# RookieJunChen/FullSubNet-plus

Hardware: AMD Instinct MI355X
Metric: STFT frames/sec (257-bin, 2 s clips), FullSubNet+ forward (higher is better)
Workload: dtype f32

## Files before the change

### fullsubnet_plus_amd/csrc/lstm.hip

```cpp
#include <cstring>

#include "fsnp_common.h"
#include "lstm_common.h"

namespace fsnp {

template <int EX>
__host__ __device__ __forceinline__ int e_frag_index(int e, int k) {
    return ((((k >> 3) * 2) + (k & 1)) * EX + e) * 4 + ((k >> 1) & 3);
}

struct WStream {
    __amdgpu_buffer_rsrc_t rsrc;
    int voff;
};
template <int NT>
__device__ __forceinline__ float4 wload(const WStream& ws, int g, int n) {
    const auto v = __builtin_amdgcn_raw_buffer_load_b128(ws.rsrc, ws.voff, (g * NT + n) * 1024, 0);
    return __builtin_bit_cast(float4, v);
}

template <int NT, int EX>
__device__ __forceinline__ void mfma_groups(f32x16 (&acc)[NT], float (&accx)[EX > 0 ? EX : 1][NT], float4 (&b)[NT],
                                            const float4* __restrict__ A, const float4* __restrict__ AE, int ngroups,
                                            const WStream& ws, int& gnext, int groups_total) {
    float4 a = A[0];
    float4 ae[EX > 0 ? EX : 1];
#pragma unroll
    for (int e = 0; e < EX; ++e) ae[e] = AE[e];
    for (int g = 0; g < ngroups; ++g) {
        const int gn = (g + 1 < ngroups ? g + 1 : g);
        const float4 an = A[gn * 64];
        float4 aen[EX > 0 ? EX : 1];
#pragma unroll
        for (int e = 0; e < EX; ++e) aen[e] = AE[gn * 2 * EX + e];
        if constexpr (EX == 0) {
#pragma unroll
            for (int n = 0; n < NT; ++n) {
                acc[n] = __builtin_amdgcn_mfma_f32_32x32x2f32(a.x, b[n].x, acc[n], 0, 0, 0);
                acc[n] = __builtin_amdgcn_mfma_f32_32x32x2f32(a.y, b[n].y, acc[n], 0, 0, 0);
                acc[n] = __builtin_amdgcn_mfma_f32_32x32x2f32(a.z, b[n].z, acc[n], 0, 0, 0);
                acc[n] = __builtin_amdgcn_mfma_f32_32x32x2f32(a.w, b[n].w, acc[n], 0, 0, 0);
                b[n] = wload<NT>(ws, gnext, n);
                __builtin_amdgcn_sched_barrier(0);
            }
        } else {
            constexpr int HALF = NT / 2;
#pragma unroll
            for (int hb = 0; hb < NT; hb += HALF) {
#pragma unroll
                for (int n = hb; n < hb + HALF; ++n) {
                    acc[n] = __builtin_amdgcn_mfma_f32_32x32x2f32(a.x, b[n].x, acc[n], 0, 0, 0);
                    acc[n] = __builtin_amdgcn_mfma_f32_32x32x2f32(a.y, b[n].y, acc[n], 0, 0, 0);
                    acc[n] = __builtin_amdgcn_mfma_f32_32x32x2f32(a.z, b[n].z, acc[n], 0, 0, 0);
                    acc[n] = __builtin_amdgcn_mfma_f32_32x32x2f32(a.w, b[n].w, acc[n], 0, 0, 0);
                }
                __builtin_amdgcn_sched_barrier(0);
#pragma unroll
                for (int n = hb; n < hb + HALF; ++n)
#pragma unroll
                    for (int e = 0; e < EX; ++e) {
                        float v = accx[e][n];
                        v = fmaf(ae[e].x, b[n].x, v);
                        v = fmaf(ae[e].y, b[n].y, v);
                        v = fmaf(ae[e].z, b[n].z, v);
                        accx[e][n] = fmaf(ae[e].w, b[n].w, v);
                    }
                __builtin_amdgcn_sched_barrier(0);
#pragma unroll
                for (int n = hb; n < hb + HALF; ++n) b[n] = wload<NT>(ws, gnext, n);
                __builtin_amdgcn_sched_barrier(0);
            }
        }
        gnext = (gnext + 1 == groups_total) ? 0 : gnext + 1;
        a = an;
#pragma unroll
        for (int e = 0; e < EX; ++e) ae[e] = aen[e];
    }
}

__device__ __forceinline__ unsigned short bf16_bits(float v) {
    const unsigned u = __float_as_uint(v);
    return (unsigned short)((u + 0x7FFFu + ((u >> 16) & 1u)) >> 16);
}
__host__ __device__ __forceinline__ int a_frag_index_bf16(int row, int k) {
    return (((k >> 4) * 64) + (((k >> 3) & 1) * 32) + row) * 8 + (k & 7);
}

template <int ST, int UW, int HBLO = 0>
__device__ __forceinline__ void lstm_cell(f32x16 (&acc)[4 * ST], f32x2 (&c)[ST][8], float* __restrict__ Hs, int wave,
                                          int lane, unsigned short* __restrict__ Hb = nullptr) {
#pragma unroll
    for (int s = 0; s < ST; ++s) {
        const int k = wave * UW + s * 32 + (lane & 31);
        const int kbase = (((k >> 3) * 64) + ((k & 1) * 32)) * 4 + ((k >> 1) & 3);
#pragma unroll
        for (int r = 0; r < 16; r += 2) {
            auto rd = [](float v) {
                if constexpr (ST > 1) { float o; asm("v_accvgpr_read_b32 %0, %1" : "=v"(o) : "a"(v)); return o; }
                else return v;
            };
            const f32x2 h = lstm_cell_pair(f32x2{rd(acc[s][r]), rd(acc[s][r + 1])}, f32x2{rd(acc[ST + s][r]), rd(acc[ST + s][r + 1])},
                                           f32x2{rd(acc[2 * ST + s][r]), rd(acc[2 * ST + s][r + 1])},
                                           f32x2{rd(acc[3 * ST + s][r]), rd(acc[3 * ST + s][r + 1])}, c[s][r >> 1]);
            const int row = (r & 3) + 8 * (r >> 2) + 4 * (lane >> 5);
            Hs[kbase + row * 4] = h.x;
            Hs[kbase + (row + 1) * 4] = h.y;
            if (Hb) {
                const unsigned short hx = bf16_bits(h.x), hy = bf16_bits(h.y);
                Hb[a_frag_index_bf16(row, k)] = hx; Hb[a_frag_index_bf16(row + 1, k)] = hy;
                if constexpr (HBLO > 0) {
                    Hb[HBLO + a_frag_index_bf16(row, k)] = bf16_bits(h.x - __uint_as_float((unsigned)hx << 16));
                    Hb[HBLO + a_frag_index_bf16(row + 1, k)] = bf16_bits(h.y - __uint_as_float((unsigned)hy << 16));
                }
            }
        }
    }
}

using bf16x8 = __attribute__((ext_vector_type(8))) __bf16;
template <int NT, int EX, int ALO>
__device__ __forceinline__ void mfma_groups_bf16(f32x16 (&acc)[NT], float (&accx)[EX > 0 ? EX : 1][NT], float4 (&b)[NT],
                                                 const float4* __restrict__ A, const float4* __restrict__ AE, int nsteps,
                                                 const WStream& ws, int& gnext, int groups_total, int lane) {
    float4 a = A[0], al = A[ALO];
    for (int g = 0; g < nsteps; ++g) {
        const float4 an = A[(g + 1 < nsteps ? g + 1 : g) * 64], aln = A[ALO + (g + 1 < nsteps ? g + 1 : g) * 64];
        float4 he[EX > 0 ? EX : 1][2];
        if constexpr (EX > 0) {
            const int kg = 2 * g + (lane >> 5);
#pragma unroll
            for (int e = 0; e < EX; ++e) { he[e][0] = AE[(kg * 2 + 0) * EX + e]; he[e][1] = AE[(kg * 2 + 1) * EX + e]; }
        }
#pragma unroll
        for (int n = 0; n < NT; ++n) {
            if constexpr (EX > 0) {
                const unsigned w0 = __float_as_uint(b[n].x), w1 = __float_as_uint(b[n].y), w2 = __float_as_uint(b[n].z),
                               w3 = __float_as_uint(b[n].w);
#pragma unroll
                for (int e = 0; e < EX; ++e) {
                    float v = accx[e][n];
                    v = fmaf(he[e][0].x, __uint_as_float(w0 << 16), v);
                    v = fmaf(he[e][1].x, __uint_as_float(w0 & 0xFFFF0000u), v);
                    v = fmaf(he[e][0].y, __uint_as_float(w1 << 16), v);
                    v = fmaf(he[e][1].y, __uint_as_float(w1 & 0xFFFF0000u), v);
                    v = fmaf(he[e][0].z, __uint_as_float(w2 << 16), v);
                    v = fmaf(he[e][1].z, __uint_as_float(w2 & 0xFFFF0000u), v);
                    v = fmaf(he[e][0].w, __uint_as_float(w3 << 16), v);
                    accx[e][n] = fmaf(he[e][1].w, __uint_as_float(w3 & 0xFFFF0000u), v);
                }
            }
            acc[n] = __builtin_amdgcn_mfma_f32_32x32x16_bf16(__builtin_bit_cast(bf16x8, a), __builtin_bit_cast(bf16x8, b[n]),
                                                             acc[n], 0, 0, 0);
            if constexpr (ALO > 0)
                acc[n] = __builtin_amdgcn_mfma_f32_32x32x16_bf16(__builtin_bit_cast(bf16x8, al), __builtin_bit_cast(bf16x8, b[n]),
                                                                 acc[n], 0, 0, 0);
            b[n] = wload<NT>(ws, gnext, n);
            __builtin_amdgcn_sched_barrier(0);
        }
        gnext = (gnext + 1 == groups_total) ? 0 : gnext + 1;
        a = an; al = aln;
    }
}

template <int ST, int UW, int EX, int NT>
__device__ __forceinline__ void lstm_cell_extra(float (&accx)[EX > 0 ? EX : 1][NT], float (&cx)[EX > 0 ? EX : 1][ST],
                                                const float* __restrict__ bias, float* __restrict__ He, int wave,
                                                int lane) {
#pragma unroll
    for (int e = 0; e < EX; ++e)
#pragma unroll
        for (int s = 0; s < ST; ++s) {
            float g4[4];
#pragma unroll
            for (int q = 0; q < 4; ++q) {
                const float v = accx[e][q * ST + s];
                g4[q] = v + __shfl_xor(v, 32) + (bias ? bias[(q * ST + s) * 32] : 0.0f);
            }
            const float cn = fast_sigmoid(g4[1]) * cx[e][s] + fast_sigmoid(g4[0]) * fast_tanh(g4[2]);
            cx[e][s] = cn;
            const float h = fast_sigmoid(g4[3]) * fast_tanh(cn);
            if (lane < 32) He[e_frag_index<EX>(e, wave * UW + s * 32 + lane)] = h;
        }
}

template <int HID, int KX, int OUT, int EX, bool PROF, int NW, bool BF>
__global__ __launch_bounds__(64 * NW) __attribute__((amdgpu_waves_per_eu(NW / 4, NW / 4)))
void lstm2_fc_kernel(LstmWeights w, LstmArgs a) {
    static_assert(OUT == 2, "FC lane mapping assumes output_size == 2");
    static_assert(EX >= 0 && EX <= 4, "at most 4 VALU rows per tile (one FC wave per extra row)");
    static_assert(NW % 4 == 0 && NW >= 4, "whole waves per SIMD");
    constexpr int NTHR = 64 * NW;
    constexpr int UW = HID / NW, ST = UW / 32, NT = 4 * ST;
    static_assert(UW % 32 == 0 && UW * NW == HID, "hidden/NW must be a multiple of 32");
    constexpr int KGX = KX / 8, KGH = HID / 8, KG0 = KGX + KGH;
    constexpr int KSB = HID / 16;
    constexpr int KG1 = BF ? KGH + KSB : 2 * KGH, KGT = KG0 + KG1;
    static_assert(KGH % 4 == 0, "FC k-split");
    static_assert(!BF || HID % 16 == 0, "bf16 k-steps");
    constexpr int RT = 32 + EX;
    constexpr int EXA = EX > 0 ? EX : 1;

    extern __shared__ __attribute__((aligned(16))) unsigned char smem_raw[];
    float4* Xs = reinterpret_cast<float4*>(smem_raw);
    float4* H0s = Xs + KGX * 64;
    float4* H1s = H0s + KGH * 64;
    float4* XEs = H1s + KGH * 64;
    float4* HE0s = XEs + KGX * 2 * EX;
    float4* HE1s = HE0s + KGH * 2 * EX;
    float4* Wfc4 = HE1s + KGH * 2 * EX;
    RowDesc* rows_s = reinterpret_cast<RowDesc*>(Wfc4 + OUT * KGH * 2);
    constexpr int BL = BF ? 1 : 2;
    constexpr bool HILO = BF && EX == 0;
    float* Bs = reinterpret_cast<float*>(rows_s + RT);
    float4* H0b = reinterpret_cast<float4*>(Bs + BL * NW * NT * 32);

    const int tid = threadIdx.x;
    const int lane = tid & 63;
    const int wave = __builtin_amdgcn_readfirstlane(tid >> 6);
    const int slot0 = blockIdx.x * RT;
    const int Tp = a.Tp;

    __shared__ unsigned long long clk_s[2];
    if (a.clk != nullptr && tid == 0) {
        clk_s[1] = __builtin_amdgcn_s_memrealtime();
        clk_s[0] = __builtin_amdgcn_s_memtime();
        if (blockIdx.x == 0) { a.clk[0] = clk_s[0]; a.clk[1] = clk_s[1]; a.clk[4] = 0ull; a.clk[5] = 0ull; a.clk[6] = ~0ull; }
    }

    for (int i = tid; i < (KGX + 2 * KGH) * (64 + 2 * EX); i += NTHR) Xs[i] = make_float4(0.f, 0.f, 0.f, 0.f);
    for (int i = tid; i < OUT * KGH * 2; i += NTHR) {
        const int o = i / (KGH * 2), kg = (i >> 1) % KGH, kh = i & 1;
        const float* wr = w.wfc + (size_t)o * HID + kg * 8 + kh;
        Wfc4[i] = make_float4(wr[0], wr[2], wr[4], wr[6]);
    }
    if (tid < RT) rows_s[tid] = a.rows[slot0 + tid];
    for (int i = tid; i < BL * NW * NT * 32; i += NTHR) {
        const int col = i & 31, n = (i >> 5) % NT, wv = (i / (32 * NT)) % NW, layer = BF ? 1 : i / (32 * NT * NW);
        Bs[i] = w.bias[layer * 4 * HID + (n / ST) * HID + wv * UW + (n % ST) * 32 + col];
    }
    __syncthreads();
    if constexpr (BF) {
        if (tid < 32) reinterpret_cast<float*>(Xs)[a_frag_index(tid, w.NIN)] = 1.0f;
        if (EX > 0 && tid < EX) reinterpret_cast<float*>(XEs)[e_frag_index<EXA>(tid, w.NIN)] = 1.0f;
    }

    const bool dense = a.dense != nullptr;
    const float* __restrict__ gbase = dense ? a.dense : a.att_mag;
    const int gstep = dense ? w.NIN : a.FP;
    auto plan = [&](const RowDesc& rd, int j) -> int {
        if (!rd.valid || j >= w.NIN) return -1;
        if (dense) return rd.b * Tp * w.NIN + j;
        return sb_feature_offset(j, rd.f, rd.b * Tp * a.FP, a.F, a.NSBN, a.NFBN, a.fb_rel, a.fb_branch_stride);
    };
    auto row_md = [&](const RowDesc& rd, int slot, NormMD& md, const NormMD*& md_row) {
        md.m = 0.0f; md.d = 1.0f; md_row = nullptr;
        if (dense || !rd.valid) return;
        if (a.md_row != nullptr) md_row = a.md_row + (size_t)slot * Tp;
        else md = a.md_utt[rd.b];
    };
    constexpr int JSTEP = NTHR / 32, NG = (KX + JSTEP - 1) / JSTEP;
    const int grow = tid & 31;
    int goff[NG], xdst[NG];
    NormMD md; const NormMD* md_row;
    {
        const RowDesc rd = rows_s[grow];
#pragma unroll
        for (int i = 0; i < NG; ++i) {
            const int j = (tid >> 5) + JSTEP * i;
            goff[i] = (j < KX && !(BF && j == w.NIN)) ? plan(rd, j) : -2;
            xdst[i] = a_frag_index(grow, j < KX ? j : 0);
        }
        row_md(rd, slot0 + grow, md, md_row);
    }
    int goffx = -1, xdstx = 0;
    NormMD mdx = {0.0f, 1.0f}; const NormMD* mdx_row = nullptr;
    bool havex = EX > 0 && tid < EX * KX;
    if (BF && havex && tid % KX == w.NIN) havex = false;
    if (havex) {
        const int e = tid / KX, j = tid % KX;
        const RowDesc rd = rows_s[32 + e];
        goffx = plan(rd, j);
        xdstx = e_frag_index<EXA>(e, j);
        row_md(rd, slot0 + 32 + e, mdx, mdx_row);
    }

    float* Xf = reinterpret_cast<float*>(Xs);
    float* XEf = reinterpret_cast<float*>(XEs);
    {
        const NormMD m0 = md_row ? md_row[0] : md;
#pragma unroll
        for (int i = 0; i < NG; ++i)
            if (goff[i] != -2) Xf[xdst[i]] = goff[i] >= 0 ? (gbase[goff[i]] - m0.m) / m0.d : 0.0f;
        if (havex) {
            const NormMD mx = mdx_row ? mdx_row[0] : mdx;
            XEf[xdstx] = goffx >= 0 ? (gbase[goffx] - mx.m) / mx.d : 0.0f;
        }
    }

    const float* __restrict__ bias_l0 = BF ? nullptr : Bs + ((0 * NW + wave) * NT) * 32 + (lane & 31);
    const float* __restrict__ bias_l1 = Bs + (((BL - 1) * NW + wave) * NT) * 32 + (lane & 31);
    f32x2 c0[ST][8], c1[ST][8];
    float cx0[EXA][ST], cx1[EXA][ST];
#pragma unroll
    for (int s = 0; s < ST; ++s) {
#pragma unroll
        for (int r = 0; r < 8; ++r) { c0[s][r] = f32x2{0.0f, 0.0f}; c1[s][r] = f32x2{0.0f, 0.0f}; }
#pragma unroll
        for (int e = 0; e < EXA; ++e) { cx0[e][s] = 0.0f; cx1[e][s] = 0.0f; }
    }

    WStream ws;
    ws.rsrc = __builtin_amdgcn_make_buffer_rsrc(const_cast<float*>(w.wpack) + (size_t)wave * KGT * NT * 256, 0,
                                                KGT * NT * 1024, 0x00020000);
    ws.voff = lane * 16;
    float4 breg[NT];
#pragma unroll
    for (int n = 0; n < NT; ++n) breg[n] = wload<NT>(ws, 0, n);
    int gnext = 1;
    auto run_groups = [&](f32x16 (&acc_)[NT], float (&accx_)[EXA][NT], const float4* A_, const float4* AE_, int ng) {
        mfma_groups<NT, EX>(acc_, accx_, breg, A_, AE_, ng, ws, gnext, KGT);
    };

    const int fc_row = (wave & 3) * 8 + (lane & 7);
    const int fc_o = (lane >> 3) & 1;
    const int fc_kp = lane >> 4;
    const RowDesc fc_rd = rows_s[fc_row];
    const RowDesc fcx_rd = (EX > 0 && wave < EX) ? rows_s[32 + (wave < EX ? wave : 0)] : RowDesc{0, 0, 0, 0};

    auto fc_store = [&](int t_of_h) {
      if (wave < 4) {
        constexpr int KGP = KGH / 4;
        float sum = 0.0f;
#pragma unroll 4
        for (int kk = 0; kk < KGP; ++kk) {
            const int kg = fc_kp * KGP + kk;
#pragma unroll
            for (int kh = 0; kh < 2; ++kh) {
                const float4 h4 = H1s[kg * 64 + kh * 32 + fc_row];
                const float4 w4 = Wfc4[(fc_o * KGH + kg) * 2 + kh];
                sum += h4.x * w4.x + h4.y * w4.y + h4.z * w4.z + h4.w * w4.w;
            }
        }
        sum += __shfl_xor(sum, 16);
        sum += __shfl_xor(sum, 32);
        if (fc_kp == 0 && fc_rd.valid && t_of_h >= a.LA)
            a.out[(size_t)fc_rd.out_off + (size_t)fc_o * a.out_stride_o + (t_of_h - a.LA)] = apply_act(sum + w.bfc[fc_o], a.act);
      }
        if (EX > 0 && wave < EX) {
            const int o = lane >> 5;
            const float* he = reinterpret_cast<const float*>(HE1s);
            float sx = 0.0f;
#pragma unroll 4
            for (int i = 0; i < HID / 32; ++i) {
                const int k = (lane & 31) + 32 * i;
                sx += he[e_frag_index<EXA>(wave, k)] * w.wfc[o * HID + k];
            }
#pragma unroll
            for (int m = 16; m > 0; m >>= 1) sx += __shfl_xor(sx, m);
            if ((lane & 31) == 0 && fcx_rd.valid && t_of_h >= a.LA)
                a.out[(size_t)fcx_rd.out_off + (size_t)o * a.out_stride_o + (t_of_h - a.LA)] = apply_act(sx + w.bfc[o], a.act);
        }
    };

    const float4* AEx = XEs + (lane >> 5) * EX;
    const float4* AEh0 = HE0s + (lane >> 5) * EX;
    const float4* AEh1 = HE1s + (lane >> 5) * EX;

    __syncthreads();

    unsigned long long* prof = nullptr;
    int prof_stride = 0;
    if constexpr (PROF) {
        const bool rec = blockIdx.x == 0 && tid == 0;
        prof = a.prof + (rec ? 0 : (size_t)Tp * 8 + (size_t)blockIdx.x * 256 + tid);
        prof_stride = rec ? 8 : 0;
    }
#define FSNP_STAMP(i) do { if constexpr (PROF) prof[t * prof_stride + (prof_stride ? (i) : 0)] = __builtin_amdgcn_s_memtime(); } while (0)

    for (int t = 0; t < Tp; ++t) {
        FSNP_STAMP(0);
        float xr[NG], xrx = 0.0f;
        NormMD mdn = md, mdxn = mdx;
        const bool have_next = (t + 1 < Tp);
        if (have_next) {
            if (md_row) mdn = md_row[t + 1];
#pragma unroll
            for (int i = 0; i < NG; ++i) xr[i] = goff[i] >= 0 ? gbase[goff[i] + (t + 1) * gstep] : 0.0f;
            if (havex) {
                if (mdx_row) mdxn = mdx_row[t + 1];
                xrx = goffx >= 0 ? gbase[goffx + (t + 1) * gstep] : 0.0f;
            }
        }

        f32x16 acc[NT];
        float accx[EXA][NT];
#pragma unroll
        for (int n = 0; n < NT; ++n) {
#pragma unroll
            for (int r = 0; r < 16; ++r) acc[n][r] = BF ? 0.0f : bias_l0[n * 32];
#pragma unroll
            for (int e = 0; e < EXA; ++e) accx[e][n] = 0.0f;
        }
        run_groups(acc, accx, Xs + lane, AEx, KG0);
        FSNP_STAMP(1);
        __syncthreads();
        FSNP_STAMP(2);
        lstm_cell<ST, UW, HILO ? KSB * 64 * 8 : 0>(acc, c0, reinterpret_cast<float*>(H0s), wave, lane, BF ? reinterpret_cast<unsigned short*>(H0b) : nullptr);
        if (EX > 0) lstm_cell_extra<ST, UW, EX, NT>(accx, cx0, bias_l0, reinterpret_cast<float*>(HE0s), wave, lane);
        if (have_next) {
#pragma unroll
            for (int i = 0; i < NG; ++i)
                if (goff[i] != -2) Xf[xdst[i]] = goff[i] >= 0 ? (xr[i] - mdn.m) / mdn.d : 0.0f;
            if (havex) XEf[xdstx] = goffx >= 0 ? (xrx - mdxn.m) / mdxn.d : 0.0f;
        }
        if (t > 0) fc_store(t - 1);
        FSNP_STAMP(3);
        __syncthreads();
        FSNP_STAMP(4);
#pragma unroll
        for (int n = 0; n < NT; ++n) {
#pragma unroll
            for (int r = 0; r < 16; ++r) acc[n][r] = bias_l1[n * 32];
#pragma unroll
            for (int e = 0; e < EXA; ++e) accx[e][n] = 0.0f;
        }
        run_groups(acc, accx, H1s + lane, AEh1, KGH);
        if constexpr (BF) mfma_groups_bf16<NT, EX, HILO ? KSB * 64 : 0>(acc, accx, breg, H0b + lane, HE0s, KSB, ws, gnext, KGT, lane);
        else run_groups(acc, accx, H0s + lane, AEh0, KGH);
        FSNP_STAMP(5);
        __syncthreads();
        FSNP_STAMP(6);
        lstm_cell<ST, UW>(acc, c1, reinterpret_cast<float*>(H1s), wave, lane);
        if (EX > 0) lstm_cell_extra<ST, UW, EX, NT>(accx, cx1, bias_l1, reinterpret_cast<float*>(HE1s), wave, lane);
        FSNP_STAMP(7);
    }
#undef FSNP_STAMP
    __syncthreads();
    fc_store(Tp - 1);
    if (a.clk != nullptr && tid == 0) {
        const unsigned long long m1 = __builtin_amdgcn_s_memtime(), r1 = __builtin_amdgcn_s_memrealtime();
        if (blockIdx.x == 0) { a.clk[2] = m1; a.clk[3] = r1; }
        atomicMax(a.clk + 4, r1 - clk_s[1]);
        atomicMax(a.clk + 5, m1 - clk_s[0]);
        atomicMin(a.clk + 6, r1 - clk_s[1]);
    }
}

size_t lstm_pack_floats(int H, int KX, int NW) {
    const int NT = 4 * (H / NW / 32);
    const int KGT = KX / 8 + H / 8 + 2 * (H / 8);
    return (size_t)NW * KGT * NT * 64 * 4;
}

void lstm_pack_weights(int H, int NIN, int KX, int NW, const float* wih0, const float* whh0, const float* wih1,
                       const float* whh1, float* wpack) {
    const int UW = H / NW, ST = UW / 32, NT = 4 * ST;
    const int KGX = KX / 8, KGH = H / 8, KG0 = KGX + KGH, KGT = KG0 + 2 * KGH;
    for (int wv = 0; wv < NW; ++wv)
        for (int g = 0; g < KGT; ++g)
            for (int n = 0; n < NT; ++n)
                for (int lane = 0; lane < 64; ++lane)
                    for (int p = 0; p < 4; ++p) {
                        const int gate = n / ST, s = n % ST;
                        const int wrow = gate * H + wv * UW + s * 32 + (lane & 31);
                        float v = 0.0f;
                        if (g < KG0) {
                            const int k = 8 * g + 2 * p + (lane >> 5);
                            if (k < KX) { if (k < NIN) v = wih0[(size_t)wrow * NIN + k]; }
                            else v = whh0[(size_t)wrow * H + (k - KX)];
                        } else {
                            const int k = 8 * (g - KG0) + 2 * p + (lane >> 5);
                            if (k < H) v = whh1[(size_t)wrow * H + k];
                            else v = wih1[(size_t)wrow * H + (k - H)];
                        }
                        wpack[((((size_t)wv * KGT + g) * NT + n) * 64 + lane) * 4 + p] = v;
                    }
}

size_t lstm_pack_floats_bf16ih(int H, int KX, int NW) {
    const int NT = 4 * (H / NW / 32);
    const int KGT = KX / 8 + H / 8 + H / 8 + H / 16;
    return (size_t)NW * KGT * NT * 64 * 4;
}

static unsigned short host_bf16(float v) {
    unsigned u;
    memcpy(&u, &v, 4);
    return (unsigned short)((u + 0x7FFFu + ((u >> 16) & 1u)) >> 16);
}

void lstm_pack_weights_bf16ih(int H, int NIN, int KX, int NW, const float* wih0, const float* whh0, const float* wih1,
                              const float* whh1, const float* bias0, float* wpack) {
    const int UW = H / NW, ST = UW / 32, NT = 4 * ST;
    const int KGX = KX / 8, KGH = H / 8, KG0 = KGX + KGH, KSB = H / 16, KGT = KG0 + KGH + KSB;
    for (int wv = 0; wv < NW; ++wv)
        for (int g = 0; g < KGT; ++g)
            for (int n = 0; n < NT; ++n)
                for (int lane = 0; lane < 64; ++lane) {
                    const int gate = n / ST, s = n % ST;
                    const int wrow = gate * H + wv * UW + s * 32 + (lane & 31);
                    float* dst = wpack + ((((size_t)wv * KGT + g) * NT + n) * 64 + lane) * 4;
                    if (g < KG0 + KGH) {
                        for (int p = 0; p < 4; ++p) {
                            float v = 0.0f;
                            if (g < KG0) {
                                const int k = 8 * g + 2 * p + (lane >> 5);
                                if (k < KX) { if (k < NIN) v = wih0[(size_t)wrow * NIN + k]; else if (k == NIN) v = bias0[wrow]; }
                                else v = whh0[(size_t)wrow * H + (k - KX)];
                            } else {
                                const int k = 8 * (g - KG0) + 2 * p + (lane >> 5);
                                v = whh1[(size_t)wrow * H + k];
                            }
                            dst[p] = v;
                        }
                    } else {
                        const int ks = g - KG0 - KGH;
                        unsigned short* d16 = reinterpret_cast<unsigned short*>(dst);
                        for (int j = 0; j < 8; ++j) d16[j] = host_bf16(wih1[(size_t)wrow * H + 16 * ks + 8 * (lane >> 5) + j]);
                    }
                }
}

template <int EX, int NW, bool BF, int KX, int HID = 384>
static void launch_lstm_ex(const LstmWeights& w, const LstmArgs& a, hipStream_t s) {
    constexpr int OUT = 2;
    constexpr int KGX = KX / 8, KGH = HID / 8, NT = 4 * (HID / NW / 32);
    const size_t smem = (size_t)(KGX + 2 * KGH) * (64 + 2 * EX) * 16 + (size_t)OUT * KGH * 2 * 16 +
                        (32 + EX) * sizeof(RowDesc) + (size_t)(BF ? 1 : 2) * NW * NT * 32 * 4 + (BF ? (size_t)(EX == 0 ? 2 : 1) * (HID / 16) * 64 * 16 : 0);
    LstmWeights wv = w;
    wv.wpack = BF ? (NW == 12 ? w.wpack_bf[1] : w.wpack_bf[0]) : (NW == 12 ? w.wpack12 : w.wpack);
    if constexpr (KX == 40 && HID == 384) {
        if (a.prof != nullptr) {
            auto kern = lstm2_fc_kernel<HID, KX, OUT, EX, true, NW, BF>;
            (void)hipFuncSetAttribute(reinterpret_cast<const void*>(kern), hipFuncAttributeMaxDynamicSharedMemorySize, (int)smem);
            hipLaunchKernelGGL(kern, dim3(a.num_tiles), dim3(64 * NW), smem, s, wv, a);
            return;
        }
    }
    auto kern = lstm2_fc_kernel<HID, KX, OUT, EX, false, NW, BF>;
    static PerDeviceOnce attr_once;
    attr_once.run([&] { (void)hipFuncSetAttribute(reinterpret_cast<const void*>(kern), hipFuncAttributeMaxDynamicSharedMemorySize, (int)smem); });
    hipLaunchKernelGGL(kern, dim3(a.num_tiles), dim3(64 * NW), smem, s, wv, a);
}

template <int NW, bool BF, int KX>
static void launch_lstm_nw(const LstmWeights& w, const LstmArgs& a, hipStream_t s) {
    switch (a.ex) {
        case 0: launch_lstm_ex<0, NW, BF, KX>(w, a, s); break;
        case 1: launch_lstm_ex<1, NW, BF, KX>(w, a, s); break;
        case 2: launch_lstm_ex<2, NW, BF, KX>(w, a, s); break;
        default: launch_lstm_ex<4, NW, BF, KX>(w, a, s); break;
    }
}

void launch_lstm(const LstmWeights& w, const LstmArgs& a, hipStream_t s) {
    if (a.num_tiles <= 0) return;
    const int waves = w.waves != 0 ? w.waves : (a.ex > 0 ? 12 : 4);
    if (w.H == 256) {
        if (w.KX == 64) launch_lstm_ex<0, 4, false, 64, 256>(w, a, s);
        else launch_lstm_ex<0, 4, false, 40, 256>(w, a, s);
        return;
    }
    if (w.KX == 64) {
        if (waves == 12) launch_lstm_nw<12, false, 64>(w, a, s);
        else launch_lstm_nw<4, false, 64>(w, a, s);
    } else if (w.ih_bf16) {
        if (waves == 12) launch_lstm_nw<12, true, 40>(w, a, s);
        else launch_lstm_nw<4, true, 40>(w, a, s);
    } else {
        if (waves == 12) launch_lstm_nw<12, false, 40>(w, a, s);
        else launch_lstm_nw<4, false, 40>(w, a, s);
    }
}

template <int ST, int UW, int HID, bool LOAD>
__device__ __forceinline__ void stream_state_io(f32x2 (&c0)[ST][8], f32x2 (&c1)[ST][8], float* __restrict__ H0, float* __restrict__ H1,
                                                const RowDesc* __restrict__ rows_s, float* __restrict__ state, long slot_stride, int done,
                                                int wave, int lane) {
#pragma unroll
    for (int r = 0; r < 16; ++r) {
        const int row = (r & 3) + 8 * (r >> 2) + 4 * (lane >> 5);
        const RowDesc rd = rows_s[row];
        const bool on = LOAD ? rd.valid > 0 : rd.valid == done;
        float* __restrict__ p = state + (size_t)rd.b * slot_stride + (size_t)rd.f * 4 * HID;
#pragma unroll
        for (int s = 0; s < ST; ++s) {
            const int k = wave * UW + s * 32 + (lane & 31);
            const int hi = (((k >> 3) * 64) + ((k & 1) * 32)) * 4 + ((k >> 1) & 3) + row * 4;
            if constexpr (LOAD) {
                H0[hi] = on ? p[k] : 0.0f;
                c0[s][r >> 1][r & 1] = on ? p[HID + k] : 0.0f;
                H1[hi] = on ? p[2 * HID + k] : 0.0f;
                c1[s][r >> 1][r & 1] = on ? p[3 * HID + k] : 0.0f;
            } else if (on) {
                p[k] = H0[hi];
                p[HID + k] = c0[s][r >> 1][r & 1];
                p[2 * HID + k] = H1[hi];
                p[3 * HID + k] = c1[s][r >> 1][r & 1];
            }
        }
    }
}

template <int HID, int KX>
__global__ __launch_bounds__(256) __attribute__((amdgpu_waves_per_eu(1, 1)))
void lstm2_fc_stream_kernel(LstmWeights w, LstmArgs a) {
    constexpr int NW = 4, NTHR = 256, OUT = 2;
    constexpr int UW = HID / NW, ST = UW / 32, NT = 4 * ST;
    constexpr int KGX = KX / 8, KGH = HID / 8, KG0 = KGX + KGH, KGT = KG0 + 2 * KGH;
    static_assert(UW % 32 == 0 && KGH % 4 == 0, "hidden/4 must be a multiple of 32");

    extern __shared__ __attribute__((aligned(16))) unsigned char smem_raw[];
    float4* Xs = reinterpret_cast<float4*>(smem_raw);
    float4* H0s = Xs + KGX * 64;
    float4* H1s = H0s + KGH * 64;
    float4* Wfc4 = H1s + KGH * 64;
    RowDesc* rows_s = reinterpret_cast<RowDesc*>(Wfc4 + OUT * KGH * 2);
    float* Bs = reinterpret_cast<float*>(rows_s + 32);

    const int tid = threadIdx.x;
    const int lane = tid & 63;
    const int wave = __builtin_amdgcn_readfirstlane(tid >> 6);
    const int slot0 = blockIdx.x * 32;
    const int Tp = a.Tp;

    for (int i = tid; i < (KGX + 2 * KGH) * 64; i += NTHR) Xs[i] = make_float4(0.f, 0.f, 0.f, 0.f);
    for (int i = tid; i < OUT * KGH * 2; i += NTHR) {
        const int o = i / (KGH * 2), kg = (i >> 1) % KGH, kh = i & 1;
        const float* wr = w.wfc + (size_t)o * HID + kg * 8 + kh;
        Wfc4[i] = make_float4(wr[0], wr[2], wr[4], wr[6]);
    }
    if (tid < 32) rows_s[tid] = a.rows[slot0 + tid];
    for (int i = tid; i < 2 * NW * NT * 32; i += NTHR) {
        const int col = i & 31, n = (i >> 5) % NT, wv = (i / (32 * NT)) % NW, layer = i / (32 * NT * NW);
        Bs[i] = w.bias[layer * 4 * HID + (n / ST) * HID + wv * UW + (n % ST) * 32 + col];
    }
    __syncthreads();

    int nsteps = 0, cmin = 1 << 30;
    for (int r = 0; r < 32; ++r) {
        const int v = rows_s[r].valid;
        nsteps = v > nsteps ? v : nsteps;
        if (v > 0) cmin = v < cmin ? v : cmin;
    }
    nsteps = __builtin_amdgcn_readfirstlane(nsteps);
    const bool mixed = __builtin_amdgcn_readfirstlane(cmin < nsteps ? 1 : 0) != 0;
    if (nsteps <= 0) return;

    constexpr int JSTEP = NTHR / 32, NG = (KX + JSTEP - 1) / JSTEP;
    const int grow = tid & 31;
    int goff[NG], xdst[NG];
    const float* __restrict__ gbase = a.att_mag;
    const int gstep = a.FP;
    const NormMD* md_row;
    {
        const RowDesc rd = rows_s[grow];
#pragma unroll
        for (int i = 0; i < NG; ++i) {
            const int j = (tid >> 5) + JSTEP * i;
            goff[i] = j >= KX ? -2 : (rd.valid > 0 && j < w.NIN)
                          ? sb_feature_offset(j, rd.f, rd.b * Tp * a.FP, a.F, a.NSBN, a.NFBN, a.fb_rel, a.fb_branch_stride) : -1;
            xdst[i] = a_frag_index(grow, j < KX ? j : 0);
        }
        md_row = a.md_row + (size_t)(slot0 + grow) * Tp;
    }
    float* Xf = reinterpret_cast<float*>(Xs);
    {
        const NormMD m0 = rows_s[grow].valid > 0 ? md_row[0] : NormMD{0.0f, 1.0f};
#pragma unroll
        for (int i = 0; i < NG; ++i)
            if (goff[i] != -2) Xf[xdst[i]] = goff[i] >= 0 ? (gbase[goff[i]] - m0.m) / m0.d : 0.0f;
    }

    const float* __restrict__ bias_l0 = Bs + ((0 * NW + wave) * NT) * 32 + (lane & 31);
    const float* __restrict__ bias_l1 = Bs + ((1 * NW + wave) * NT) * 32 + (lane & 31);
    f32x2 c0[ST][8], c1[ST][8];
    stream_state_io<ST, UW, HID, true>(c0, c1, reinterpret_cast<float*>(H0s), reinterpret_cast<float*>(H1s), rows_s, a.st_sb, a.st_stride, 0,
                                       wave, lane);

    WStream ws;
    ws.rsrc = __builtin_amdgcn_make_buffer_rsrc(const_cast<float*>(w.wpack) + (size_t)wave * KGT * NT * 256, 0, KGT * NT * 1024, 0x00020000);
    ws.voff = lane * 16;
    float4 breg[NT];
#pragma unroll
    for (int n = 0; n < NT; ++n) breg[n] = wload<NT>(ws, 0, n);
    int gnext = 1;
    float accx[1][NT];
    auto run_groups = [&](f32x16 (&acc_)[NT], const float4* A_, int ng) {
        mfma_groups<NT, 0>(acc_, accx, breg, A_, A_, ng, ws, gnext, KGT);
    };

    const int fc_row = (wave & 3) * 8 + (lane & 7);
    const int fc_o = (lane >> 3) & 1;
    const int fc_kp = lane >> 4;
    const RowDesc fc_rd = rows_s[fc_row];
    auto fc_store = [&](int t_of_h) {
        constexpr int KGP = KGH / 4;
        float sum = 0.0f;
#pragma unroll 4
        for (int kk = 0; kk < KGP; ++kk) {
            const int kg = fc_kp * KGP + kk;
#pragma unroll
            for (int kh = 0; kh < 2; ++kh) {
                const float4 h4 = H1s[kg * 64 + kh * 32 + fc_row];
                const float4 w4 = Wfc4[(fc_o * KGH + kg) * 2 + kh];
                sum += h4.x * w4.x + h4.y * w4.y + h4.z * w4.z + h4.w * w4.w;
            }
        }
        sum += __shfl_xor(sum, 16);
        sum += __shfl_xor(sum, 32);
        if (fc_kp == 0 && t_of_h < fc_rd.valid)
            a.out[(size_t)fc_rd.out_off + (size_t)fc_o * a.out_stride_o + t_of_h] = apply_act(sum + w.bfc[fc_o], a.act);
    };

    __syncthreads();

    for (int t = 0; t < nsteps; ++t) {
        float xr[NG];
        NormMD mdn = {0.0f, 1.0f};
        const bool have_next = (t + 1 < nsteps);
        if (have_next) {
            if (rows_s[grow].valid > 0) mdn = md_row[t + 1];
#pragma unroll
            for (int i = 0; i < NG; ++i) xr[i] = goff[i] >= 0 ? gbase[goff[i] + (t + 1) * gstep] : 0.0f;
        }

        f32x16 acc[NT];
#pragma unroll
        for (int n = 0; n < NT; ++n)
#pragma unroll
            for (int r = 0; r < 16; ++r) acc[n][r] = bias_l0[n * 32];
        run_groups(acc, Xs + lane, KG0);
        __syncthreads();
        lstm_cell<ST, UW>(acc, c0, reinterpret_cast<float*>(H0s), wave, lane);
        if (have_next) {
#pragma unroll
            for (int i = 0; i < NG; ++i)
                if (goff[i] != -2) Xf[xdst[i]] = goff[i] >= 0 ? (xr[i] - mdn.m) / mdn.d : 0.0f;
        }
        if (t > 0) fc_store(t - 1);
        __syncthreads();
#pragma unroll
        for (int n = 0; n < NT; ++n)
#pragma unroll
            for (int r = 0; r < 16; ++r) acc[n][r] = bias_l1[n * 32];
        run_groups(acc, H1s + lane, KGH);
        run_groups(acc, H0s + lane, KGH);
        __syncthreads();
        lstm_cell<ST, UW>(acc, c1, reinterpret_cast<float*>(H1s), wave, lane);
        if (t + 1 == nsteps || mixed)
            stream_state_io<ST, UW, HID, false>(c0, c1, reinterpret_cast<float*>(H0s), reinterpret_cast<float*>(H1s), rows_s, a.st_sb,
                                                a.st_stride, t + 1, wave, lane);
    }
    __syncthreads();
    fc_store(nsteps - 1);
}

template <int HID, int KX>
static void launch_lstm_stream_one(const LstmWeights& w, const LstmArgs& a, hipStream_t s) {
    constexpr int KGX = KX / 8, KGH = HID / 8, NT = 4 * (HID / 4 / 32);
    const size_t smem = (size_t)(KGX + 2 * KGH) * 64 * 16 + (size_t)2 * KGH * 2 * 16 + 32 * sizeof(RowDesc) + (size_t)2 * 4 * NT * 32 * 4;
    auto kern = lstm2_fc_stream_kernel<HID, KX>;
    static PerDeviceOnce attr_once;
    attr_once.run([&] { (void)hipFuncSetAttribute(reinterpret_cast<const void*>(kern), hipFuncAttributeMaxDynamicSharedMemorySize, (int)smem); });
    hipLaunchKernelGGL(kern, dim3(a.num_tiles), dim3(256), smem, s, w, a);
}

bool lstm_stream_available(const LstmWeights& w) {
    return !w.gru && w.OUT == 2 && (w.H == 384 || w.H == 256) && (w.KX == 40 || w.KX == 64) && w.wpack != nullptr;
}

void launch_lstm_stream(const LstmWeights& w, const LstmArgs& a, hipStream_t s) {
    if (a.num_tiles <= 0) return;
    if (w.H == 256) { if (w.KX == 64) launch_lstm_stream_one<256, 64>(w, a, s); else launch_lstm_stream_one<256, 40>(w, a, s); }
    else if (w.KX == 64) launch_lstm_stream_one<384, 64>(w, a, s);
    else launch_lstm_stream_one<384, 40>(w, a, s);
}

LstmPlan plan_lstm_tiles(int num_rows, int num_cus) {
    LstmPlan p{};
    if (num_rows <= 32 * num_cus) {
        p.ex = 0; p.num_tiles = cdiv(num_rows, 32);
    } else {
        const int cand[4] = {0, 1, 2, 4};
        int best_rounds = 1 << 30;
        for (int i = 0; i < 4; ++i) {
            const int rounds = cdiv(cdiv(num_rows, 32 + cand[i]), num_cus);
            if (rounds < best_rounds) { best_rounds = rounds; p.ex = cand[i]; }
        }
        p.num_tiles = best_rounds * num_cus;
    }
    p.rows_per_slot_tile = 32 + p.ex;
    return p;
}

}
```

Baseline: 147,200.

## Skip zero-padded input K-groups in LSTM MFMA passes and skip zero h0 at t=0

Replaces the generic rotating MFMA group loop with explicit passes that compute only the input K-groups actually occupied by NIN features, issuing a partial group for the remainder. At the first timestep it also skips the recurrent H contributions, which are known zero. Weight prefetch indices are remapped so the streamed B fragments follow the new irregular group order. This cuts wasted MFMAs and weight loads on padded columns, at the cost of more complex index logic and the risk of mismatched weight/activation groups.

New measurement: 147,100 (median of 5 runs). Within noise of the previous version (-0.1%).

```diff
diff --git a/fullsubnet_plus_amd/csrc/lstm.hip b/fullsubnet_plus_amd/csrc/lstm.hip
--- a/fullsubnet_plus_amd/csrc/lstm.hip
+++ b/fullsubnet_plus_amd/csrc/lstm.hip
@@ -77,6 +77,55 @@
 #pragma unroll
         for (int e = 0; e < EX; ++e) ae[e] = aen[e];
     }
+}
+
+template <int NT>
+__device__ __forceinline__ void mfma_group(f32x16 (&acc)[NT], float4 (&b)[NT], const float4& a, const WStream& ws, int gload) {
+#pragma unroll
+    for (int n = 0; n < NT; ++n) {
+        acc[n] = __builtin_amdgcn_mfma_f32_32x32x2f32(a.x, b[n].x, acc[n], 0, 0, 0);
+        acc[n] = __builtin_amdgcn_mfma_f32_32x32x2f32(a.y, b[n].y, acc[n], 0, 0, 0);
+        acc[n] = __builtin_amdgcn_mfma_f32_32x32x2f32(a.z, b[n].z, acc[n], 0, 0, 0);
+        acc[n] = __builtin_amdgcn_mfma_f32_32x32x2f32(a.w, b[n].w, acc[n], 0, 0, 0);
+        b[n] = wload<NT>(ws, gload, n);
+        __builtin_amdgcn_sched_barrier(0);
+    }
+}
+template <int NT>
+__device__ __forceinline__ void mfma_group_part(f32x16 (&acc)[NT], float4 (&b)[NT], const float4& a, const WStream& ws, int gload,
+                                                int live) {
+#pragma unroll
+    for (int n = 0; n < NT; ++n) {
+        acc[n] = __builtin_amdgcn_mfma_f32_32x32x2f32(a.x, b[n].x, acc[n], 0, 0, 0);
+        if (live > 1) acc[n] = __builtin_amdgcn_mfma_f32_32x32x2f32(a.y, b[n].y, acc[n], 0, 0, 0);
+        if (live > 2) acc[n] = __builtin_amdgcn_mfma_f32_32x32x2f32(a.z, b[n].z, acc[n], 0, 0, 0);
+        if (live > 3) acc[n] = __builtin_amdgcn_mfma_f32_32x32x2f32(a.w, b[n].w, acc[n], 0, 0, 0);
+        b[n] = wload<NT>(ws, gload, n);
+        __builtin_amdgcn_sched_barrier(0);
+    }
+}
+template <int NT, class GroupOf, class AidxOf>
+__device__ __forceinline__ void mfma_pass(f32x16 (&acc)[NT], float4 (&b)[NT], float4& a, const float4* __restrict__ A, int ibeg,
+                                          int iend, GroupOf group_of, AidxOf aidx_of, const WStream& ws) {
+    int i = ibeg;
+    {
+        typedef float f32x4_t __attribute__((ext_vector_type(4)));
+        f32x4_t v = {a.x, a.y, a.z, a.w};
+        asm volatile("" : "+v"(v));
+        a = make_float4(v.x, v.y, v.z, v.w);
+    }
+    do {
+        const float4 an = A[aidx_of(i + 1) * 64];
+        mfma_group<NT>(acc, b, a, ws, group_of(i + 1));
+        a = an;
+    } while (++i < iend);
+}
+
+__device__ __forceinline__ void x_live_steps(int NIN, int KX, int& xsteps, int& xlive) {
+    const int nin = NIN < 1 ? 1 : (NIN > KX ? KX : NIN);
+    const int groups = (nin + 7) >> 3, rem = nin - 8 * (groups - 1);
+    xsteps = groups < 2 ? 2 : groups;
+    xlive = groups < 2 ? 1 : (rem + 1) >> 1;
 }
 
 __device__ __forceinline__ unsigned short bf16_bits(float v) {
@@ -321,6 +370,11 @@
     auto run_groups = [&](f32x16 (&acc_)[NT], float (&accx_)[EXA][NT], const float4* A_, const float4* AE_, int ng) {
         mfma_groups<NT, EX>(acc_, accx_, breg, A_, AE_, ng, ws, gnext, KGT);
     };
+    constexpr bool PASSES = EX == 0 && !BF;
+    int xsteps = KGX, xlive = 4;
+    if constexpr (PASSES) x_live_steps(w.NIN, KX, xsteps, xlive);
+    auto l1_group = [&](int i) { return i < 2 * KGH ? KG0 + i : 0; };
+    auto l1_aidx = [&](int i) { return i < KGH ? KG0 + i : KGX - KGH + i; };
 
     const int fc_row = (wave & 3) * 8 + (lane & 7);
     const int fc_o = (lane >> 3) & 1;
@@ -402,7 +456,17 @@
 #pragma unroll
             for (int e = 0; e < EXA; ++e) accx[e][n] = 0.0f;
         }
-        run_groups(acc, accx, Xs + lane, AEx, KG0);
+        if constexpr (PASSES) {
+            const int l0_h = t > 0 ? KGH : 1, l0_next = t > 0 ? KG0 : KG0 + KGH;
+            auto l0_aidx = [&](int i) { return i < xsteps ? i : i + (KGX - xsteps); };
+            auto l0_group = [&](int i) { return i < xsteps + l0_h ? l0_aidx(i) : l0_next; };
+            float4 av = Xs[lane];
+            mfma_pass<NT>(acc, breg, av, Xs + lane, 0, xsteps - 1, l0_group, l0_aidx, ws);
+            const float4 ah = H0s[lane];
+            mfma_group_part<NT>(acc, breg, av, ws, KGX, xlive);
+            av = ah;
+            mfma_pass<NT>(acc, breg, av, Xs + lane, xsteps, xsteps + l0_h, l0_group, l0_aidx, ws);
+        } else run_groups(acc, accx, Xs + lane, AEx, KG0);
         FSNP_STAMP(1);
         __syncthreads();
         FSNP_STAMP(2);
@@ -425,9 +489,15 @@
 #pragma unroll
             for (int e = 0; e < EXA; ++e) accx[e][n] = 0.0f;
         }
-        run_groups(acc, accx, H1s + lane, AEh1, KGH);
-        if constexpr (BF) mfma_groups_bf16<NT, EX, HILO ? KSB * 64 : 0>(acc, accx, breg, H0b + lane, HE0s, KSB, ws, gnext, KGT, lane);
-        else run_groups(acc, accx, H0s + lane, AEh0, KGH);
+        if constexpr (PASSES) {
+            const int l1_beg = t > 0 ? 0 : KGH;
+            float4 av = Xs[lane + l1_aidx(l1_beg) * 64];
+            mfma_pass<NT>(acc, breg, av, Xs + lane, l1_beg, 2 * KGH, l1_group, l1_aidx, ws);
+        } else {
+            run_groups(acc, accx, H1s + lane, AEh1, KGH);
+            if constexpr (BF) mfma_groups_bf16<NT, EX, HILO ? KSB * 64 : 0>(acc, accx, breg, H0b + lane, HE0s, KSB, ws, gnext, KGT, lane);
+            else run_groups(acc, accx, H0s + lane, AEh0, KGH);
+        }
         FSNP_STAMP(5);
         __syncthreads();
         FSNP_STAMP(6);
@@ -685,11 +755,11 @@
     float4 breg[NT];
 #pragma unroll
     for (int n = 0; n < NT; ++n) breg[n] = wload<NT>(ws, 0, n);
-    int gnext = 1;
-    float accx[1][NT];
-    auto run_groups = [&](f32x16 (&acc_)[NT], const float4* A_, int ng) {
-        mfma_groups<NT, 0>(acc_, accx, breg, A_, A_, ng, ws, gnext, KGT);
-    };
+    int xsteps, xlive;
+    x_live_steps(w.NIN, KX, xsteps, xlive);
+    auto l0_aidx = [&](int i) { return i < xsteps ? i : i + (KGX - xsteps); };
+    auto l1_group = [&](int i) { return i < 2 * KGH ? KG0 + i : 0; };
+    auto l1_aidx = [&](int i) { return i < KGH ? KG0 + i : KGX - KGH + i; };
 
     const int fc_row = (wave & 3) * 8 + (lane & 7);
     const int fc_o = (lane >> 3) & 1;
@@ -731,7 +801,12 @@
         for (int n = 0; n < NT; ++n)
 #pragma unroll
             for (int r = 0; r < 16; ++r) acc[n][r] = bias_l0[n * 32];
-        run_groups(acc, Xs + lane, KG0);
+        float4 av = Xs[lane];
+        mfma_pass<NT>(acc, breg, av, Xs + lane, 0, xsteps - 1, l0_aidx, l0_aidx, ws);
+        const float4 ah = H0s[lane];
+        mfma_group_part<NT>(acc, breg, av, ws, KGX, xlive);
+        av = ah;
+        mfma_pass<NT>(acc, breg, av, Xs + lane, xsteps, xsteps + KGH, l0_aidx, l0_aidx, ws);
         __syncthreads();
         lstm_cell<ST, UW>(acc, c0, reinterpret_cast<float*>(H0s), wave, lane);
         if (have_next) {
@@ -745,8 +820,8 @@
         for (int n = 0; n < NT; ++n)
 #pragma unroll
             for (int r = 0; r < 16; ++r) acc[n][r] = bias_l1[n * 32];
-        run_groups(acc, H1s + lane, KGH);
-        run_groups(acc, H0s + lane, KGH);
+        av = H1s[lane];
+        mfma_pass<NT>(acc, breg, av, Xs + lane, 0, 2 * KGH, l1_group, l1_aidx, ws);
         __syncthreads();
         lstm_cell<ST, UW>(acc, c1, reinterpret_cast<float*>(H1s), wave, lane);
         if (t + 1 == nsteps || mixed)
```
